# tphakala/go-audio-resampler

Hardware: AMD Instinct MI355X
Metric: Msamples/s resampled (float32, 44.1k→48k QualityHigh) + RMS error vs Go ref (higher is better)
Workload: dtype f32

## Files before the change

go-audio-resampler_amd/csrc/gar_hxs.hip:

```cpp
#include <hip/hip_runtime.h>

#include <algorithm>
#include <cstdio>
#include <cstdlib>
#include <utility>
#include <vector>

#include "gar_hxt.hpp"

namespace gar {

#define GAR_HXS_EXT(NS, V) extern template hipError_t hxsLaunch<NS, V>(const HxsArgs&, size_t, int64_t, hipStream_t);
GAR_HXS_FOR_ALL(GAR_HXS_EXT)
#undef GAR_HXS_EXT
#define GAR_HXT_EXT(NS, F, V, L) extern template hipError_t hxtLaunch<NS, F, V, L>(const HxsArgs&, size_t, int64_t, hipStream_t);
GAR_HXT_FOR_A(GAR_HXT_EXT)
GAR_HXT_FOR_B(GAR_HXT_EXT)
#undef GAR_HXT_EXT

namespace {
constexpr int kProfWords = 64 + 2 * 4096;
unsigned long long* profBuf() {
    static unsigned long long* p = nullptr;
    static bool init = false;
    if (!init) {
        init = true;
        if (std::getenv("GAR_HXS_PROF") && hipMalloc(&p, kProfWords * sizeof(unsigned long long)) == hipSuccess) {
            (void)hipMemset(p, 0, kProfWords * sizeof(unsigned long long));
            (void)hipMemset(p + 10, 0xff, sizeof(unsigned long long));
            (void)hipMemset(p + 13, 0xff, sizeof(unsigned long long));
            std::atexit([] {
                static unsigned long long h[kProfWords] = {};
                if (hipDeviceSynchronize() == hipSuccess && hipMemcpy(h, p, sizeof(h), hipMemcpyDeviceToHost) == hipSuccess) {
                    const double nl = h[3] ? static_cast<double>(h[3]) : 1, nc = h[6] ? static_cast<double>(h[6]) : 1;
                    fprintf(stderr, "hxs prof per wave (cycles): loaders convert %.0f issue+wait %.0f (issue %.0f) barrier %.0f (life %.1f us) | compute convert+mfma %.0f barrier %.0f\n",
                            h[0] / nl, h[1] / nl, h[7] / nl, h[2] / nl, h[9] / nl / 100.0, h[4] / nc, h[5] / nc);
                    fprintf(stderr, "hxs loader pre-loop %.2f us, post-loop %.2f us; compute convert %.0f\n", h[8] / nl / 100.0, h[12] / nl / 100.0, h[15] / nc);
                    if (h[23]) fprintf(stderr, "hxs wave-0 first block (cycles): entry->window %.0f, window->steps done %.0f, ->exit (stores drained) %.0f, n %llu\n",
                                       static_cast<double>(h[20]) / h[23], static_cast<double>(h[21]) / h[23], static_cast<double>(h[22]) / h[23], h[23]);
                    if (h[23]) fprintf(stderr, "hxs wave-0: entry->A landed %.0f, entry->barrier 1 %.0f; wave entry spread in a workgroup %.0f, wave 0 after first wave %.0f\n",
                                       static_cast<double>(h[24]) / h[23], static_cast<double>(h[25]) / h[23], static_cast<double>(h[26]) / h[23], static_cast<double>(h[27]) / h[23]);
                    if (h[34]) fprintf(stderr, "hxt roles per block (cycles): compute wave 0 %.0f (waiting %.0f), loader 0 %.0f (waiting %.0f), n %llu\n",
                                       static_cast<double>(h[30]) / h[34], static_cast<double>(h[32]) / h[34], static_cast<double>(h[31]) / h[34],
                                       static_cast<double>(h[33]) / h[34], h[34]);
                    if (h[34]) fprintf(stderr, "hxt compute wave 0: entry -> first group %.0f cycles, last group -> exit %.0f cycles, periods %.0f, arrivals %.0f\n",
                                       static_cast<double>(h[35]) / h[34], static_cast<double>(h[36]) / h[34],
                                       static_cast<double>(h[37]) / h[34], static_cast<double>(h[38]) / h[34]);
                    if (h[34] && h[57]) fprintf(stderr, "hxt fill (cycles): entry -> A issued %.0f, -> fill barrier %.0f, -> first group %.0f; in-kernel clock %.3f GHz\n",
                                       static_cast<double>(h[53]) / h[34], static_cast<double>(h[54]) / h[34], static_cast<double>(h[55]) / h[34],
                                       0.1 * static_cast<double>(h[56]) / static_cast<double>(h[57]));
                    if (h[34]) fprintf(stderr, "hxt loader 0 phases (cycles): load data wait %.0f, conversion %.0f, arrival %.0f\n",
                                       static_cast<double>(h[50]) / h[34], static_cast<double>(h[51]) / h[34], static_cast<double>(h[52]) / h[34]);
                    if (h[44]) fprintf(stderr, "hxq wave 0 (cycles): entry->barrier 1 %.0f, ->image %.0f, ->MFMA+stores issued %.0f, ->drained %.0f, n %llu\n",
                                       static_cast<double>(h[40]) / h[44], static_cast<double>(h[41]) / h[44], static_cast<double>(h[42]) / h[44],
                                       static_cast<double>(h[43]) / h[44], h[44]);
                    fprintf(stderr, "hxs span: first start -> last end %.1f us; loader wave life min %.1f max %.1f us\n",
                            (h[11] - h[10]) / 100.0, h[13] / 100.0, h[14] / 100.0);
                    std::vector<std::pair<double, int>> v;
                    unsigned long long t0 = ~0ull;
                    for (int b = 0; b < 4096; ++b)
                        if (h[65 + 2 * b]) { v.push_back({h[65 + 2 * b] / 100.0, b}); t0 = std::min(t0, h[64 + 2 * b]); }
                    if (!v.empty()) {
                        std::vector<std::pair<double, int>> sv = v;
                        std::sort(sv.begin(), sv.end());
                        auto pc = [&](double q) { return sv[std::min(sv.size() - 1, static_cast<size_t>(q * sv.size()))].first; };
                        fprintf(stderr, "hxs WG life us: n %zu min %.1f p10 %.1f p50 %.1f p90 %.1f max %.1f |", sv.size(), sv.front().first, pc(0.1), pc(0.5), pc(0.9), sv.back().first);
                        for (int m = 0; m < 8; ++m) {
                            double s = 0; int n = 0;
                            for (auto& e : v) if (e.second % 8 == m) { s += e.first; ++n; }
                            fprintf(stderr, " x%d %.1f", m, n ? s / n : 0.0);
                        }
                        fprintf(stderr, "\n  slowest:");
                        for (size_t k = sv.size(); k-- > 0 && k + 8 >= sv.size();)
                            fprintf(stderr, " b%d %.1fus@+%.1f", sv[k].second, sv[k].first, (h[64 + 2 * sv[k].second] - t0) / 100.0);
                        fprintf(stderr, "\n");
                    }
                }
            });
        }
    }
    return p;
}

int64_t fdiv(int64_t a, int64_t b) { return a >= 0 ? a / b : -((-a + b - 1) / b); }
int64_t cdiv(int64_t a, int64_t b) { return -fdiv(-a, b); }

template <int NS, int NL>
hipError_t hxtFmtL(const HxsArgs& x, size_t lds, int64_t blocks, hipStream_t st) {
    if (x.fmt == 1 && x.vst == 2) return hxtLaunch<NS, 1, 2, NL>(x, lds, blocks, st);
    if (x.fmt == 2 && x.vst == 0) return hxtLaunch<NS, 2, 0, NL>(x, lds, blocks, st);
    if (x.fmt == 2 && x.vst == 1) return hxtLaunch<NS, 2, 1, NL>(x, lds, blocks, st);
    if (x.fmt == 5 && x.vst == 0) return hxtLaunch<NS, 5, 0, NL>(x, lds, blocks, st);
    return hipErrorNotSupported;
}
template <int NS>
hipError_t hxtFmt(const HxsArgs& x, size_t lds, int64_t blocks, hipStream_t st) {
    return x.ncomp + 6 <= kHxtWaves ? hxtFmtL<NS, 6>(x, lds, blocks, st) : hxtFmtL<NS, 4>(x, lds, blocks, st);
}

static int hxtRoles(int nprog, int NS, int* role, int* maxStride) {
    static const int knobRoles = std::getenv("GAR_HXT_ROLES") ? std::atoi(std::getenv("GAR_HXT_ROLES")) : -1;
    const bool balanced = knobRoles >= 0 ? knobRoles != 0 : NS >= 10;
    int w = 0;
    *maxStride = 1;
    if (!balanced) {
        for (int i = 0; i < nprog; ++i) role[w++] = i | (1 << 16);
        return w;
    }
    const int q = nprog / 4 * 4, r = nprog - q;
    for (int i = 0; i < q; ++i) role[w++] = i | (1 << 16);
    if (r == 2 && q + 4 <= kHxtMaxComp) {
        for (int i = 0; i < 4; ++i) role[w++] = (q + (i & 1)) | ((i >> 1) << 8) | (2 << 16);
        *maxStride = 2;
    } else if (r == 1 && q + 4 <= kHxtMaxComp) {
        for (int i = 0; i < 4; ++i) role[w++] = q | (i << 8) | (4 << 16);
        *maxStride = 4;
    } else {
        for (int i = q; i < nprog; ++i) role[w++] = i | (1 << 16);
    }
    return w;
}

template <int NS>
hipError_t hxsVst(const HxsArgs& x, size_t lds, int64_t blocks, hipStream_t st) {
    switch (x.vst) {
        case 0: return hxsLaunch<NS, 0>(x, lds, blocks, st);
        case 1: return hxsLaunch<NS, 1>(x, lds, blocks, st);
        case 2: return hxsLaunch<NS, 2>(x, lds, blocks, st);
        case 4: return hxsLaunch<NS, 4>(x, lds, blocks, st);
        default: return hxsLaunch<NS, 3>(x, lds, blocks, st);
    }
}
}

static_assert(kHxtSyncOff + kHxtSyncBytes <= 320, "hxt progress counters past the reserved LDS");
static size_t hxsLds(int Rt) { return 4 * (16 * static_cast<size_t>(Rt) + 64) + 320; }
static_assert(288 + kHxtSyncBytes <= 448, "hxt FMT 5 progress counters past the reserved LDS");
static size_t hxtLdsWide(int Rt) { return 8 * (16 * static_cast<size_t>(Rt) + 64) + 448; }

static void hxsRingFor(const HxDev& p, int G, int& R, int& Rt, int& Wg) {
    const int GQ = G * p.Qc;
    Wg = (G - 1) * p.Qc + p.Kread;
    const int n = (Wg + GQ + GQ - 1) / GQ;
    R = n * GQ;
    Rt = (R + std::max(0, Wg - GQ) + 15) / 16 * 16;
}
constexpr size_t kHxsStaticLds = kHxsDev ? sizeof(unsigned long long) * kHxsWaves : 0;
static bool hxsRingFits(const HxDev& p, int G, int Rt) {
    return hxsLds(Rt) + kHxsStaticLds <= 160 * 1024 && (G * p.Qc + 63) / 64 <= kHxsNP;
}

static bool hxsNsBuilt(int ns) { return GAR_HXS_QUICK ? (ns == 9 || ns == 10) : (ns >= 1 && ns <= 10); }

bool hxsPlanFits(const HxDev& p) {
    if (!p.rb || p.nw > kHxRbMaxWaves || !hxsNsBuilt(p.NS)) return false;
// ... 31 lines not shown
        hxsRingFor(p, 2, r2, rt2, wg2);
        wide = ms == 1 && hxtLdsWide(rt2) <= 160 * 1024 && 2 * Qc <= hxtMaxRowsF(5, nc + 6 <= kHxtWaves ? 6 : 4) &&
               r2 / (2 * static_cast<int>(Qc)) + 3 <= kHxtSlots;
    }
    const int bw = wide ? 32 : 16;
    const int64_t targetBlocks = static_cast<int64_t>(ncu) * (knobWg > 0 ? knobWg : 1);
    const int64_t nchunkT = small ? nmac : std::max<int64_t>(1, (targetBlocks * bw + C - 1) / C);
    int64_t Np = std::max<int64_t>(1, cdiv(nmac, nchunkT));
    static const int knobNp = std::getenv("GAR_HXS_NP") ? std::atoi(std::getenv("GAR_HXS_NP")) : 0;
    if (knobNp > 0 && !small) Np = knobNp;
    const int inEsz = src.in_pcm ? pcmBytes(src.in_pcm) : (src.in_f64 ? 8 : 4);
    const int64_t rowBytes = std::max<int64_t>(4, src.in_fs * inEsz);
    const int64_t chunksPerRsrc = (C <= 16 && 16 % C == 0) ? 16 / C : 1;
    const int64_t npMax = ((int64_t(1) << 31) / rowBytes / chunksPerRsrc - (3 * Qc + p.Kread + 256)) / Qc;
    const bool rawSpan = npMax >= 1;
    if (rawSpan) Np = std::min(Np, npMax);
    int64_t nchunk = cdiv(nmac, Np);
    if (16 % C == 0 && !small) nchunk = cdiv(nchunk * C, 16) * 16 / C;
    const int64_t ncols = nchunk * C;
    if (ncols > (int64_t(1) << 30) || Np > (int64_t(1) << 24)) return hipErrorNotSupported;

    const uintptr_t inA = reinterpret_cast<uintptr_t>(src.in);
    int fmt = 0;
    const bool stereoIl = C == 2 && src.in_fs == 2 && src.in_cs == 1;
    if (!src.in) {
        const uintptr_t hA = reinterpret_cast<uintptr_t>(src.hist);
        if (C == 2 && src.hist_ld == 2 && (hA & 7) == 0) fmt = 1;
        else if (C % 16 == 0 && src.hist_ld % 4 == 0 && (hA & 15) == 0) fmt = 2;
    } else if (src.in_pcm == 16) {
        if ((inA & 3) == 0 && stereoIl) fmt = 3;
    } else if (src.in_pcm) {
        if ((inA & 7) == 0 && stereoIl) fmt = 4;
    } else if (src.in_f64) {
    } else if ((inA & 7) == 0 && stereoIl) {
        fmt = 1;
    } else if ((inA & 15) == 0 && C % 16 == 0 && src.in_cs == 1 && src.in_fs % 4 == 0) {
        fmt = 2;
    }
    const int esz = od.pcm ? pcmBytes(od.pcm) : (od.f64 ? 8 : 4);
    char* const outBase = reinterpret_cast<char*>(reinterpret_cast<uintptr_t>(od.out) - static_cast<uintptr_t>(od.o0 * od.fs * esz));
    const bool al = (reinterpret_cast<uintptr_t>(outBase) & 15) == 0;
    int vst;
    if (od.pcm == 16 && al && C == 2 && od.fs == 2 && od.cs == 1 && Pc % 4 == 0) vst = 4;
    else if (od.pcm) vst = 0;
    else if (od.f64) vst = 3;
    else if (al && C == 2 && od.fs == 2 && od.cs == 1 && Pc % 4 == 0) vst = 2;
    else if (al && od.fs == 1 && (od.cs * 4) % 16 == 0 && Pc % 4 == 0) vst = 1;
    else vst = 0;

    static const int knobHxt = std::getenv("GAR_HXT") ? std::atoi(std::getenv("GAR_HXT")) : -1;
    int role[kHxtMaxComp] = {}, maxStride = 1, ncomp = 0;
    bool hxt = knobHxt != 0 && !small && !od.pcm && !od.f64 && !src.in_pcm &&
               ((fmt == 1 && vst == 2) || (fmt == 2 && (vst == 0 || vst == 1)));
    if (hxt) ncomp = hxtRoles(p.nw, p.NS, role, &maxStride);
    wide = wide && hxt && fmt == 2 && vst == 0;
    if (wide) fmt = 5;

    int G = 0, R = 0, Rt = 0, Wg = 0;
    auto pickG = [&]() {
        for (int pass = hxt && maxStride > 1 ? 0 : 1; pass < 2 && G == 0; ++pass) {
            for (int cand = small ? 1 : kHxsMaxG; cand >= 1; --cand) {
                int r, rt, wg;
                hxsRingFor(p, cand, r, rt, wg);
                if (cand > 1 && cand > Np) continue;
                if (knobG > 0 && cand > knobG && cand > 1) continue;
                if (fmt == 5 ? hxtLdsWide(rt) > 160 * 1024 : !hxsRingFits(p, cand, rt)) continue;
                if (hxt && cand * Qc > hxtMaxRowsF(fmt, ncomp + 6 <= kHxtWaves ? 6 : 4)) continue;
                if (hxt && r / (cand * static_cast<int>(Qc)) + 3 > kHxtSlots) continue;
                if (pass == 0 && cand % maxStride != 0) continue;
                G = cand; R = r; Rt = rt; Wg = wg;
                break;
            }
        }
    };
    pickG();
    if (fmt == 5 && (G < 2 || maxStride > 1)) {
        fmt = 2;
        G = 0;
        pickG();
    }
    if (G == 0 && hxt) {
        hxt = false;
        ncomp = 0;
        maxStride = 1;
        for (int& r : role) r = 0;
        pickG();
    }
    if (G == 0) return hipErrorNotSupported;

    HxsArgs x{};
    x.A = static_cast<const h8v*>(p.A);
    x.progs = p.progs;
    x.ea = p.ea;
    x.Pc = p.Pc; x.Qc = p.Qc; x.Kc = p.Kc; x.Kread = p.Kread; x.G = G; x.C = C;
    x.nprog = p.nw;
    x.ncols = static_cast<int>(ncols);
    x.nblocks = static_cast<int>(fmt == 5 ? (ncols + 31) / 32 : (ncols + 15) / 16);
    x.Np = static_cast<int>(Np);
    x.ngroups = static_cast<int>(cdiv(Np, G));
    x.R = R; x.Rt = Rt; x.mirror = std::max(0, Wg - G * static_cast<int>(Qc)); x.Wg = Wg;
    x.a_lo = a_lo; x.a_hi = a_hi;
    x.dbg = knobDbg;
    x.prof = profBuf();
    x.o_lo = od.o_lo; x.o_hi = od.o_hi;
    const bool rawOk = src.in && fmt != 0 && src.in_len > 0 && src.in_fs > 0 && src.in_cs >= 0 && rawSpan;
    x.in_esz = inEsz;
    x.in_pcm = src.in_pcm;
    x.in = reinterpret_cast<const char*>(reinterpret_cast<uintptr_t>(src.in) -
                                         static_cast<uintptr_t>(src.in_base * src.in_fs * inEsz));
    x.in_fs = src.in_fs;
    x.in_cs = src.in_cs;
    x.fastLo = rawOk ? src.in_base : 0;
    x.fastHi = rawOk ? std::min(src.in_base + src.in_len, src.valid_end) : 0;
    x.fmt = fmt;
    x.small = small ? 1 : 0;
    static const int knobSmallK = std::getenv("GAR_HXS_SMALLK") ? std::atoi(std::getenv("GAR_HXS_SMALLK")) : 1;
    x.bigSmall = knobSmallK ? 0 : 1;
    static const int knobNt = std::getenv("GAR_HXS_NT") ? std::atoi(std::getenv("GAR_HXS_NT")) : 0;
    static const int knobPair = std::getenv("GAR_HXS_PAIR") ? std::atoi(std::getenv("GAR_HXS_PAIR")) : 1;
    x.nt = knobNt;
    x.xcdPair = knobPair && fmt == 2 && (C / 16) % 2 == 0 && x.nblocks % 16 == 0 ? 1 : 0;
    static const int knobChunkMajor = std::getenv("GAR_HXT_CHUNKMAJOR") ? std::atoi(std::getenv("GAR_HXT_CHUNKMAJOR")) : 1;
    if (knobChunkMajor && fmt == 5 && x.nblocks % 8 == 0) x.xcdPair = 2;
    x.out_pcm = od.pcm;
    x.out_f64 = od.f64;
    x.out = outBase;
    x.out_fs = od.fs * esz;
    x.out_cs = od.cs * esz;
    x.vst = vst;
    x.ncomp = ncomp;
    for (int w = 0; w < kHxtMaxComp; ++w) x.role[w] = role[w];
    x.err = od.err;
    x.pollMax = 1 << 24;
    x.faultNeed = 0;
    static const int knobCoop = std::getenv("GAR_HXT_COOP") ? std::atoi(std::getenv("GAR_HXT_COOP")) : 2;
    x.coop = std::max(0, std::min(2, knobCoop));
    if (hxt) {
        const char* f = std::getenv("GAR_HXT_FAULT");
        if (f && f[0] == '1') {
            x.pollMax = 1 << 12;
            x.faultNeed = 1 << 28;
        }
    }
    x.src = src;
    x.od = od;
    x.rows = p.rows;
    x.rowOff = p.rowOff;
    x.rowLen = p.rowLen;
    x.rowMax = p.rowMax;
    x.twoStage = p.twoStage;
    x.rowPh = p.rowPh;
    x.rowPar = p.rowPar;
    x.polyA = p.polyA;
    x.dftC = p.dftC;
    x.T1 = p.T1;
    x.T2 = p.T2;
    if (trace)
        fprintf(stderr, "%s: small=%d o[%lld,%lld) C=%d G=%d Np=%lld ngroups=%d nblocks=%d R=%d Rt=%d Wg=%d fmt=%d vst=%d fast[%lld,%lld)\n",
                hxt ? "hxt" : "hxs", x.small, (long long)od.o_lo, (long long)od.o_hi, C, G, (long long)Np, x.ngroups, x.nblocks, R, Rt, Wg, x.fmt, x.vst,
                (long long)x.fastLo, (long long)x.fastHi);
    if (hc && hc->n > 0 && hc->dst) {
        x.hdst = static_cast<float*>(hc->dst);
        x.ht0 = hc->t0;
        x.hn = hc->n;
        hc->done = true;
    }
    static const int knobHxq = std::getenv("GAR_HXQ") ? std::atoi(std::getenv("GAR_HXQ")) : 1;
    static const int knobHxqNr = std::getenv("GAR_HXQ_NR") ? std::atoi(std::getenv("GAR_HXQ_NR")) : 0;
    {
        const uintptr_t hA = reinterpret_cast<uintptr_t>(src.hist);
        const int hAl = fmt == 1 ? 8 : (fmt == 2 ? 16 : 4), hLd = fmt == 1 ? 2 : (fmt == 2 ? 4 : 1);
        const bool histOk = !src.hist || src.hist_len <= 0 ||
                            ((hA % hAl) == 0 && src.hist_ld % hLd == 0 && src.hist_len * src.hist_ld * 4 < (int64_t(1) << 31));
        const int64_t spanRows = (16 / C + 2) * Np * Qc + Wg;
        const bool gen = fmt == 0 && !src.in_pcm && src.in_fs >= 0 && src.in_cs >= 0 &&
                         (spanRows * src.in_fs + static_cast<int64_t>(C) * src.in_cs) * inEsz < (int64_t(1) << 31);
        const bool hkOk = !hc || hc->n <= 0 || (hc->n * src.in_fs + static_cast<int64_t>(C) * src.in_cs) * inEsz < (int64_t(1) << 31);
        if (small && knobHxq && ((fmt == 1 || fmt == 2) ? rawSpan : gen) && histOk && hkOk && p.nw <= 12 && x.Np == 1) {
            int nr = 1;
            for (int cand = p.nw; cand >= 1; --cand)
                if (x.nblocks * static_cast<int64_t>(cdiv(p.nw, cand)) >= static_cast<int64_t>(ncu)) { nr = cand; break; }
            if (knobHxqNr > 0) nr = std::min(knobHxqNr, p.nw);
            static const int knobOpt = std::getenv("GAR_HXQ_OPT") ? std::atoi(std::getenv("GAR_HXQ_OPT")) : 1;
            x.qOpt = knobOpt;
            x.qRbs = nr;
            x.qGroups = static_cast<int>(cdiv(p.nw, nr));
            for (int w = 0; w < p.nw; ++w) { x.qU0[w] = p.hU0[w]; x.qRbw[w] = p.hRbw[w]; }
            if (fmt == 0) {
                x.fastLo = src.in ? src.in_base : 0;
                x.fastHi = src.in ? std::min(src.in_base + src.in_len, src.valid_end) : 0;
            }
        }
    }
    if (small && !x.bigSmall) {
        Rt = R = (Wg + 15) / 16 * 16;
        x.R = R; x.Rt = Rt; x.mirror = 0;
    }
    if (trace && x.qGroups > 0) fprintf(stderr, "hxq: qRbs=%d qGroups=%d workgroups=%lld\n", x.qRbs, x.qGroups, (long long)x.nblocks * x.qGroups);
    const size_t lds = fmt == 5 ? hxtLdsWide(Rt) : hxsLds(Rt);
    const int64_t blocks = x.nblocks;
    if (hxt) {
        const int64_t hblocks = blocks;
        switch (p.NS) {
#define GAR_HXT_NS(n) case n: return hxtFmt<n>(x, lds, hblocks, stream);
#if !GAR_HXS_QUICK
            GAR_HXT_NS(1) GAR_HXT_NS(2) GAR_HXT_NS(3) GAR_HXT_NS(4) GAR_HXT_NS(5) GAR_HXT_NS(6) GAR_HXT_NS(7)
            GAR_HXT_NS(8)
#endif
            GAR_HXT_NS(9) GAR_HXT_NS(10)
#undef GAR_HXT_NS
            default: return hipErrorNotSupported;
        }
    }
    switch (p.NS) {
#define GAR_HXS_NS(n) case n: return hxsVst<n>(x, lds, blocks, stream);
#if !GAR_HXS_QUICK
        GAR_HXS_NS(1) GAR_HXS_NS(2) GAR_HXS_NS(3) GAR_HXS_NS(4) GAR_HXS_NS(5) GAR_HXS_NS(6) GAR_HXS_NS(7)
        GAR_HXS_NS(8)
#endif
        GAR_HXS_NS(9) GAR_HXS_NS(10)
#undef GAR_HXS_NS
        default: return hipErrorNotSupported;
    }
}

}
```

go-audio-resampler_amd/csrc/gar_hxt.hpp:

```cpp
#pragma once
#include "gar_hxs.hpp"

namespace gar {

constexpr int kHxtMaxComp = 12;
constexpr int kHxtWaves = 16;
constexpr int kHxtD = 2;
__host__ __device__ constexpr int hxtPieces(int NL) { return NL >= 6 ? 12 : 10; }
__host__ __device__ constexpr int hxtMaxRows(int NL) { return 64 * hxtPieces(NL); }
template <int NL>
constexpr int hxtItems() { return (4 * hxtPieces(NL) + NL - 1) / NL; }
__host__ __device__ constexpr int hxtQuads(int FMT) { return FMT == 5 ? 8 : 4; }
__host__ __device__ constexpr int hxtCols(int FMT) { return 4 * hxtQuads(FMT); }
__host__ __device__ constexpr int hxtMaxRowsF(int FMT, int NL) {
    return FMT == 5 ? 8 * NL * ((4 * hxtPieces(NL) + NL - 1) / NL) : 64 * hxtPieces(NL);
}
#ifndef GAR_HXT_CPRIO
#define GAR_HXT_CPRIO 0
#endif
#ifndef GAR_HXT_LPRIO
#define GAR_HXT_LPRIO 0
#endif
#ifndef GAR_HXT_CTDBG
#define GAR_HXT_CTDBG 0
// ... 284 lines not shown
    const int W = x.fmt == 5 ? 32 : 16;
    const bool blockLive = (x.fmt == 1 || x.fmt == 2 || x.fmt == 5) && b * W + W - 1 < x.ncols && x.fastHi > x.fastLo;
    const int64_t row0 = (x.a_lo + static_cast<int64_t>((b * W) / x.C) * x.Np) * x.Qc;
    return blockLive && row0 >= x.fastLo;
}

template <int FMT, int kCoopB, bool kOrdered>
__device__ __forceinline__ void hxtCoopStage0(const HxsArgs& x, const HxsShared& sh, int b, int w, int nw, int lane) {
    const HxsArgsP xp = hxsCold();
    const HxsRegSrc rs = hxsRegSrc<FMT>(xp, b, lane);
    HxsStage st;
    st.T0 = 0;
    st.nrow = x.Wg;
    st.fast = true;
    const int Wg = x.Wg;
    const int nit = FMT == 1 ? 4 * ((Wg + 63) >> 6) : FMT == 5 ? (Wg + 7) >> 3 : (Wg + 15) >> 4;
    bool met = !kOrdered;
    for (int it0 = w; it0 < nit; it0 += kCoopB * nw) {
        f32x4 e[kCoopB];
#pragma unroll
        for (int u = 0; u < kCoopB; ++u) {
            const int it = it0 + u * nw;
            const bool on = it < nit;
            if constexpr (FMT == 1) {
                const int q = it & 3, pc = it >> 2;
                const int o = on ? rs.lane0 + 64 * pc * rs.rowB + 2 * q * rs.chunkB : kHxqOob;
                const int o2 = on ? o + rs.chunkB : kHxqOob;
                const f2v a = __builtin_bit_cast(f2v, __builtin_amdgcn_raw_buffer_load_b64(rs.r, o, 0, 0));
                const f2v c = __builtin_bit_cast(f2v, __builtin_amdgcn_raw_buffer_load_b64(rs.r, o2, 0, 0));
                e[u] = f32x4{a.x, a.y, c.x, c.y};
            } else {
                const int o = on ? rs.lane0 + (FMT == 5 ? 8 : 16) * it * rs.rowB : kHxqOob;
                e[u] = __builtin_bit_cast(f32x4, __builtin_amdgcn_raw_buffer_load_b128(rs.r, o, 0, 0));
            }
        }
        if (!met) {
            hxsBarrier();
            met = true;
        }
#pragma unroll
        for (int u = 0; u < kCoopB; ++u) {
            const int it = it0 + u * nw;
            if (it >= nit) continue;
            const int q = FMT == 1 ? (it & 3) : FMT == 5 ? (lane & 7) : (lane >> 4);
            const int row = FMT == 1 ? 64 * (it >> 2) + lane : FMT == 5 ? 8 * it + (lane >> 3) : 16 * it + (lane & 15);
            if (row < Wg) hxsPutItem(xp, st, 0, q, row, e[u], sh.ring, sh.QS, sh.loudLo, sh.loudHi, sh.flag);
        }
    }
    if (!met) hxsBarrier();
}

template <int FMT, int NL>
__device__ __forceinline__ void hxtLoaders(const HxsArgs& x, const HxsShared& sh, const HxtSync& sy, int b, int l,
                                           int lane, int coop, unsigned long long* waited) {
    if constexpr (GAR_HXT_LPRIO > 0) __builtin_amdgcn_s_setprio(GAR_HXT_LPRIO);
    const HxsArgsP xp = hxsCold();
    const int GQ = x.G * x.Qc, Wg = x.Wg, R = x.R;
    const int P = (Wg + GQ - 1) / GQ, nL = P + x.ngroups - 1;
    const int nstepsPad = hxsStepsPad(x);
    const int dbg = kHxsDev ? x.dbg : GAR_HXT_CTDBG;
    const int c1 = b * hxtCols(FMT) + hxtCols(FMT) - 1;
    const bool blockLive = x.fmt >= 1 && x.fmt <= 5 && c1 < x.ncols && x.fastHi > x.fastLo;
    const int64_t row0 = (x.a_lo + static_cast<int64_t>((b * hxtCols(FMT)) / x.C) * x.Np) * x.Qc;
    const int64_t fastLo = x.fastLo;
    auto stage = [&](int j) {
        HxsStage st;
        st.T0 = j < P ? j * GQ : Wg + (j - P) * GQ;
        st.nrow = j < P ? min(GQ, Wg - j * GQ) : GQ;
        st.fast = blockLive && row0 + st.T0 >= fastLo;
        return st;
    };
    HxtBuf<FMT, NL> buf[kHxtD];
    bool fastL[kHxtD];
    const HxsRegSrc rs = hxsRegSrc<FMT>(xp, b, lane);
    const int jStart = coop ? P : 0;
    if (coop == 2) {
        hxsBarrier();
        fastL[0] = hxtIssue<FMT, NL>(stage(jStart), jStart < nL, rs, l, buf[0]);
        hxsBarrier();
#pragma unroll
        for (int d = 1; d < kHxtD; ++d) fastL[d] = hxtIssue<FMT, NL>(stage(jStart + d), jStart + d < nL, rs, l, buf[d]);
    } else {
#pragma unroll
        for (int d = 0; d < kHxtD; ++d) fastL[d] = hxtIssue<FMT, NL>(stage(jStart + d), jStart + d < nL, rs, l, buf[d]);
        if (coop) hxsBarrier();
    }
    int p0 = coop ? Wg : 0, last = Wg + GQ - 1 - R, need = 0;
    for (int j0 = jStart; j0 < nstepsPad; j0 += kHxtD) {
#pragma unroll
        for (int d = 0; d < kHxtD; ++d) {
            const int j = j0 + d;
            if (j < nL) {
                if (j >= P) {
                    if (j == P) p0 = Wg;
                    need = last < 0 ? 0 : need + 1;
                    if (need > 0 && !(dbg & 64)) hxtWait(x, sy, sy.cpArr, need - 1, x.ncomp, kHxtErrSlotWait, lane, waited);
                    last += GQ;
                }
                const bool stp = kHxsDev && waited;
                unsigned long long t1 = stp ? __builtin_amdgcn_s_memtime() : 0;
                if (stp && fastL[d]) {
                    constexpr int kNewer = (FMT == 1 ? 2 : 1) * hxtItems<NL>() * (kHxtD - 1);
                    static_assert(kNewer < 64, "vmcnt field");
                    __builtin_amdgcn_s_waitcnt((kNewer & 15) | (7 << 4) | (15 << 8) | ((kNewer >> 4) << 14));
                    const unsigned long long t2 = __builtin_amdgcn_s_memtime();
                    waited[3] += t2 - t1;
                    t1 = t2;
                }
                if (!((dbg & 16) && j >= P)) {
                    const HxsStage st = stage(j);
                    if (fastL[d]) hxtConvert<FMT, NL>(x, st, uni(p0), buf[d], b, l, lane, sh);
                    else hxtGatherLoad<hxtQuads(FMT)>(xp, st, b, l, NL, lane, sh);
                }
                unsigned long long t3 = stp ? __builtin_amdgcn_s_memtime() : 0;
                if (stp) waited[4] += t3 - t1;
                hxtArrive(sy.ldArr, j, lane);
                if (stp) waited[5] += __builtin_amdgcn_s_memtime() - t3;
                p0 += GQ;
                if (p0 >= R) p0 -= R;
            }
            fastL[d] = hxtIssue<FMT, NL>(stage(j + kHxtD), j + kHxtD < nL && !((dbg & 1) && j >= P), rs, l, buf[d]);
        }
    }
}

__device__ __forceinline__ int hxtBlock(const HxsArgs& x, int i) {
    if (x.xcdPair == 2) return (i & 7) * (x.nblocks >> 3) + (i >> 3);
    return hxsBlock(x, i);
}

#ifndef GAR_HXT_NTST2
#define GAR_HXT_NTST2 1
#endif
__device__ __forceinline__ void hxtStoreStereoNt(char* p, const f32x4& y, int lane) {
    const bool even = (lane & 1) == 0;
    const float s0 = even ? y[2] : y[0], s1 = even ? y[3] : y[1];
    const float q0 = __int_as_float(__builtin_amdgcn_mov_dpp(__float_as_int(s0), 0xB1, 0xf, 0xf, false));
    const float q1 = __int_as_float(__builtin_amdgcn_mov_dpp(__float_as_int(s1), 0xB1, 0xf, 0xf, false));
    f32x4 w;
    if (even) { w[0] = y[0]; w[1] = q0; w[2] = y[1]; w[3] = q1; }
    else      { w[0] = q0; w[1] = y[2]; w[2] = q1; w[3] = y[3]; }
    __builtin_nontemporal_store(w, reinterpret_cast<f32x4*>(p));
}

template <int NS, int VST, bool FAST, int NT = 1>
__device__ __forceinline__ void hxtGroups(const HxsArgs& x, const HxsShared& sh_, const HxtSync& sy, int wt, int lane,
                                          const h8v (&Ah)[NS], const h8v (&Al)[NS], uint32_t laneOff, int u0, int P,
                                          int nslot, const HxtRole& ro, char* obase, int64_t pstride, int64_t aCol,
                                          int64_t oRow0, bool colOk, int ccol, bool fullRb, int nl, unsigned long long* st) {
    const int sh = -(x.ea + kHxXs);
    const int GQ = x.G * x.Qc;
    const uint32_t dL = 8u * static_cast<uint32_t>(x.Rt);
    const uint32_t pst = 8u * static_cast<uint32_t>(x.Qc) * static_cast<uint32_t>(ro.st);
    const int dbg = kHxsDev ? x.dbg : GAR_HXT_CTDBG;
    const uint32_t tileLds = 4u * sh_.QS;
    const int64_t tileOut = 16 * x.out_cs;
    auto epilogue = [&](const f32x4& oA, const f32x4& oL, int p, int h) {
        const f32x4 y = hxScale(oA, oL, sh);
        if (dbg & 2) return;
        if constexpr (FAST && VST == 2 && GAR_HXT_NTST2) {
            hxtStoreStereoNt(obase + static_cast<int64_t>(p) * pstride, y, lane);
        } else if constexpr (FAST) {
            hxsStoreFast<VST>(x, obase + static_cast<int64_t>(p) * pstride + h * tileOut, y, lane);
        } else {
            const int ccol_ = ccol + 16 * h;
            const int64_t a = aCol + p;
            const int64_t o0 = a * x.Pc + oRow0;
            const bool live = colOk && a < x.a_hi;
            if (fullRb && live && a * x.Pc >= x.o_lo && (a + 1) * x.Pc <= x.o_hi) {
                char* pp = x.out + (o0 + ((VST == 2 && (lane & 1)) ? 2 : 0)) * x.out_fs + (VST == 2 ? 0 : ccol_ * x.out_cs);
                hxsStoreFast<VST>(x, pp, y, lane);
            } else if (live) {
#pragma unroll
                for (int i = 0; i < 4; ++i) {
                    const int64_t o = o0 + i;
                    if (oRow0 + i < x.Pc && o >= x.o_lo && o < x.o_hi)
                        *reinterpret_cast<float*>(x.out + o * x.out_fs + ccol_ * x.out_cs) = y[i];
                }
            }
        }
    };
    int first = ro.ph;
    for (int g = 0; g < x.ngroups; ++g) {
        const int p0 = g * x.G;
        const int pend = min(p0 + x.G, x.Np);
        while (first < p0) first += ro.st;
        const int n = first >= pend ? 0 : (pend - first + ro.st - 1) / ro.st;
        if (n > 0) {
            if (!(dbg & 32)) hxtWait(x, sy, sy.ldArr, P + g - 1 + x.faultNeed, nl, kHxtErrLoadWait, lane, st);
            if (kHxsDev && st) {
                const unsigned long long tg = __builtin_amdgcn_s_memtime();
                if (st[1] == 0) st[1] = tg;
                st[5] = tg;
            }
            int ln = lane;
            asm volatile("" : "+v"(ln));
            const uint32_t lo = ((ln & 15) & 3) * sh_.QS + 8u * (4 * (ln >> 4) + ((ln & 15) >> 2));
            uint32_t aH = static_cast<uint32_t>(reinterpret_cast<uintptr_t>((lds_s4p)(sh_.ring))) + lo + 8u * static_cast<uint32_t>(u0) +
                          8u * static_cast<uint32_t>((g % nslot) * GQ) + 8u * static_cast<uint32_t>(x.Qc) * static_cast<uint32_t>(first - p0);
            h8v bh0 = (dbg & 8) ? h8v{} : bFragA(aH), bl0 = (dbg & 8) ? h8v{} : bFragA(aH + dL);
            for (int i = 0; i < n; ++i) {
#pragma unroll
              for (int h = 0; h < NT; ++h) {
                asm volatile("" : "+v"(aH));
                const bool last = i + 1 == n && h + 1 == NT;
                uint32_t aL = aH + dL;
#if GAR_HXT_LOBASE
                asm volatile("" : "+v"(aL));
#endif
                const uint32_t aN = h + 1 < NT ? aH + tileLds : aH - (NT - 1) * tileLds + pst, aNL = aN + dL;
                f32x4 nA = {0, 0, 0, 0}, nL = nA;
#pragma unroll
                for (int s = 0; s < NS; ++s) {
// ... 23 lines not shown
        if (kHxsDev && st && n > 0) st[3] += ta - st[5];
        hxtArrive(sy.cpArr, g, lane);
        if (kHxsDev && st) st[4] += __builtin_amdgcn_s_memtime() - ta;
    }
    if (kHxsDev && st) st[2] = __builtin_amdgcn_s_memtime();
}

template <int NS, int VST, int FMT>
__device__ __forceinline__ void hxtCompute(const HxsArgs& x, const HxsShared& sh_, const HxtSync& sy, int b, int wt,
                                           int lane, int nl, int coop, unsigned long long* st) {
    if constexpr (GAR_HXT_CPRIO > 0) __builtin_amdgcn_s_setprio(GAR_HXT_CPRIO);
    const HxtRole ro = hxtRole(x, wt);
    const int* pt = x.progs + kBgProgInts * ro.rb;
    const int u0 = uni(pt[4]), rbw = uni(pt[3]);
    h8v Ah[NS], Al[NS];
#pragma unroll
    for (int i = 0; i < NS; ++i) {
        Ah[i] = x.A[((static_cast<size_t>(ro.rb) * NS + i) * 2 + 0) * 64 + lane];
        Al[i] = x.A[((static_cast<size_t>(ro.rb) * NS + i) * 2 + 1) * 64 + lane];
    }
    if (kHxsDev && st) st[6] = __builtin_amdgcn_s_memtime();
    if (coop) {
        if (coop == 2) hxtCoopStage0<FMT, 4, true>(x, sh_, b, wt, x.ncomp, lane);
        else hxtCoopStage0<FMT, 4, false>(x, sh_, b, wt, x.ncomp, lane);
        hxsBarrier();
    }
    if (kHxsDev && st) st[7] = __builtin_amdgcn_s_memtime();
    const uint32_t QS = sh_.QS;
    const int GQ = x.G * x.Qc;
    const int grp = lane >> 4, l16 = lane & 15;
    const uint32_t laneOff = (l16 & 3) * QS + 8u * (4 * grp + (l16 >> 2));
    const bool fullRb = (rbw + 1) * 16 <= x.Pc;
    const int nslot = x.R / GQ;
    const int P = (x.Wg + GQ - 1) / GQ;
    const int64_t pstride = static_cast<int64_t>(x.Pc) * x.out_fs;
    const int col = b * hxtCols(FMT) + l16;
    const bool colOk = col < x.ncols;
    const int kcol = col / x.C, ccol = col - kcol * x.C;
    const int64_t aCol = x.a_lo + static_cast<int64_t>(kcol) * x.Np;
    const int64_t oRow0 = static_cast<int64_t>(rbw) * 16 + 4 * grp;
    const bool laneFast = fullRb && colOk && aCol + x.Np <= x.a_hi && aCol * x.Pc >= x.o_lo &&
                          (aCol + x.Np) * x.Pc <= x.o_hi;
    char* obase = x.out + (aCol * x.Pc + oRow0 + ((VST == 2 && (lane & 1)) ? 2 : 0)) * x.out_fs +
                  (VST == 2 ? 0 : ccol * x.out_cs);
    constexpr int NT = FMT == 5 ? 2 : 1;
    if (__builtin_amdgcn_ballot_w64(!laneFast) == 0)
        hxtGroups<NS, VST, true, NT>(x, sh_, sy, wt, lane, Ah, Al, laneOff, u0, P, nslot, ro, obase, pstride, aCol, oRow0,
                                     colOk, ccol, fullRb, nl, st);
    else
        hxtGroups<NS, VST, false, NT>(x, sh_, sy, wt, lane, Ah, Al, laneOff, u0, P, nslot, ro, obase, pstride, aCol, oRow0,
                                      colOk, ccol, fullRb, nl, st);
}

template <int NS, int FMT, int VST, int NL>
__global__ __launch_bounds__(64 * kHxtWaves) void hxt_kernel(HxsArgs x) {
    extern __shared__ __attribute__((aligned(16))) unsigned char smem[];
    HxsShared s;
    s.stamp = nullptr;
    s.QS = 16u * static_cast<uint32_t>(x.Rt) + 64u;
    s.ring = reinterpret_cast<char*>(smem);
    constexpr int NQ = hxtQuads(FMT), NC = hxtCols(FMT);
    s.loudLo = reinterpret_cast<int*>(smem + NQ * static_cast<size_t>(s.QS));
    s.loudHi = s.loudLo + NC;
    s.flag = s.loudHi + NC;
    HxtSync sy;
    sy.ldArr = (lds_i32*)(smem + NQ * static_cast<size_t>(s.QS) + hxtSyncOff(FMT));
    sy.cpArr = sy.ldArr + kHxtSlots;
    sy.abort = sy.cpArr + kHxtSlots;
    const int lane = threadIdx.x & 63;
    const int wt = uni(threadIdx.x >> 6);
    const bool comp = wt < x.ncomp;
    if (threadIdx.x == 0) *sy.abort = 0;
    const bool stampW = kHxsDev && x.prof && lane == 0 && (wt == 0 || wt == x.ncomp);
    const unsigned long long tEntry = stampW ? __builtin_amdgcn_s_memtime() : 0;
    const unsigned long long rEntry = stampW ? __builtin_amdgcn_s_memrealtime() : 0;
    unsigned long long st[8] = {0, 0, 0, 0, 0, 0, 0, 0};
    unsigned long long tBlockEnd = 0;
    for (int bi = blockIdx.x; bi < x.nblocks; bi += gridDim.x) {
        const int b = hxtBlock(x, bi);
        __syncthreads();
        if (threadIdx.x < NC) {
            s.loudLo[threadIdx.x] = INT_MAX;
            s.loudHi[threadIdx.x] = -1;
        }
        const int GQb = x.G * x.Qc, Pb = (x.Wg + GQb - 1) / GQb;
        const int coop = hxtStage0Fast(x, b) ? x.coop : 0;
        if (threadIdx.x < 2 * kHxtSlots) sy.ldArr[threadIdx.x] = (coop && static_cast<int>(threadIdx.x) < Pb) ? NL : 0;
        if (threadIdx.x == 64) *s.flag = 0;
        __syncthreads();
        const bool first = bi == static_cast<int>(blockIdx.x);
        unsigned long long* stp = (stampW && first) ? st : nullptr;
        if (comp) hxtCompute<NS, VST, FMT>(x, s, sy, b, wt, lane, NL, coop, stp);
        else hxtLoaders<FMT, NL>(x, s, sy, b, wt - x.ncomp, lane, coop, stp);
        if (stampW && first) tBlockEnd = __builtin_amdgcn_s_memtime();
        __syncthreads();
        if (*s.flag) {
            __builtin_amdgcn_s_waitcnt(0);
            __syncthreads();
            hxsFixup(hxsCold(), (NC / 16) * b, s.loudLo, s.loudHi);
            if constexpr (NC == 32) hxsFixup(hxsCold(), 2 * b + 1, s.loudLo + 16, s.loudHi + 16);
        }
    }
    if (x.hn > 0) hxsHistKeep(x, static_cast<int64_t>(blockIdx.x) * blockDim.x + threadIdx.x,
                              static_cast<int64_t>(gridDim.x) * blockDim.x);
    if (stampW) {
        __builtin_amdgcn_s_waitcnt(0);
        const unsigned long long tExit = __builtin_amdgcn_s_memtime(), rExit = __builtin_amdgcn_s_memrealtime();
        if (wt == 0) {
            atomicAdd(x.prof + 30, tBlockEnd - tEntry);
            atomicAdd(x.prof + 32, st[0]);
            atomicAdd(x.prof + 37, st[3]);
            atomicAdd(x.prof + 38, st[4]);
            atomicAdd(x.prof + 34, 1ull);
            atomicAdd(x.prof + 35, st[1] ? st[1] - tEntry : 0ull);
            atomicAdd(x.prof + 36, tExit - (st[2] ? st[2] : tExit));
            atomicAdd(x.prof + 53, st[6] - tEntry);
            atomicAdd(x.prof + 54, st[7] - st[6]);
            atomicAdd(x.prof + 55, st[1] ? st[1] - st[7] : 0ull);
            atomicAdd(x.prof + 56, tExit - tEntry);
            atomicAdd(x.prof + 57, rExit - rEntry);
            atomicMin(x.prof + 10, rEntry);
            atomicMax(x.prof + 11, rExit);
            if (blockIdx.x < 4096) { x.prof[64 + 2 * blockIdx.x] = rEntry; x.prof[65 + 2 * blockIdx.x] = rExit - rEntry; }
        } else {
            atomicAdd(x.prof + 31, tBlockEnd - tEntry);
            atomicAdd(x.prof + 33, st[0]);
            atomicAdd(x.prof + 50, st[3]);
            atomicAdd(x.prof + 51, st[4]);
            atomicAdd(x.prof + 52, st[5]);
        }
    }
}

template <int NS, int FMT, int VST, int NL>
hipError_t hxtLaunch(const HxsArgs& x, size_t lds, int64_t blocks, hipStream_t st) {
    if (x.ncomp + NL > kHxtWaves) return hipErrorInvalidConfiguration;
    if (const size_t lim_ = setMaxLdsOnce(reinterpret_cast<const void*>(&hxt_kernel<NS, FMT, VST, NL>)); lim_ < lds) return ldsTooBig("hxt_kernel", lds, lim_);
    hipLaunchKernelGGL((hxt_kernel<NS, FMT, VST, NL>), dim3(static_cast<unsigned>(blocks)), dim3(64 * (x.ncomp + NL)), lds,
                       st, x);
    return hipGetLastError();
}

#define GAR_HXT_FOR3(M, NS) M(NS, 1, 2, 4) M(NS, 2, 0, 4) M(NS, 2, 1, 4) M(NS, 1, 2, 6) M(NS, 2, 0, 6) M(NS, 2, 1, 6) \
    M(NS, 5, 0, 4) M(NS, 5, 0, 6)
#if GAR_HXS_QUICK
#define GAR_HXT_FOR_A(M) GAR_HXT_FOR3(M, 9)
#define GAR_HXT_FOR_B(M) GAR_HXT_FOR3(M, 10)
#else
#define GAR_HXT_FOR_A(M) GAR_HXT_FOR3(M, 1) GAR_HXT_FOR3(M, 2) GAR_HXT_FOR3(M, 3) GAR_HXT_FOR3(M, 4) GAR_HXT_FOR3(M, 5) \
    GAR_HXT_FOR3(M, 6) GAR_HXT_FOR3(M, 7)
#define GAR_HXT_FOR_B(M) GAR_HXT_FOR3(M, 8) GAR_HXT_FOR3(M, 9) GAR_HXT_FOR3(M, 10)
#endif
#define GAR_HXT_INST(NS, F, V, L) template hipError_t hxtLaunch<NS, F, V, L>(const HxsArgs&, size_t, int64_t, hipStream_t);

}
```

Measured before the change: 454,800.

## Add compile-time specialized lean loader path for stereo f32 QualityHigh geometry

```diff
diff --git a/go-audio-resampler_amd/csrc/gar_hxs.hip b/go-audio-resampler_amd/csrc/gar_hxs.hip
--- a/go-audio-resampler_amd/csrc/gar_hxs.hip
+++ b/go-audio-resampler_amd/csrc/gar_hxs.hip
@@ -17,6 +17,9 @@
 GAR_HXT_FOR_A(GAR_HXT_EXT)
 GAR_HXT_FOR_B(GAR_HXT_EXT)
 #undef GAR_HXT_EXT
+#define GAR_HXT_EXT_LEAN(NS, F, V, L, E) extern template hipError_t hxtLaunch<NS, F, V, L, E>(const HxsArgs&, size_t, int64_t, hipStream_t);
+GAR_HXT_FOR_LEAN(GAR_HXT_EXT_LEAN)
+#undef GAR_HXT_EXT_LEAN
 
 namespace {
 constexpr int kProfWords = 64 + 2 * 4096;
@@ -86,7 +89,9 @@
 int64_t cdiv(int64_t a, int64_t b) { return -fdiv(-a, b); }
 
 template <int NS, int NL>
-hipError_t hxtFmtL(const HxsArgs& x, size_t lds, int64_t blocks, hipStream_t st) {
+hipError_t hxtFmtL(const HxsArgs& x, size_t lds, int64_t blocks, hipStream_t st, bool lean) {
+    if constexpr (NS == kHxtLeanNS)
+        if (lean && x.fmt == 1 && x.vst == 2) return hxtLaunch<NS, 1, 2, NL, 1>(x, lds, blocks, st);
     if (x.fmt == 1 && x.vst == 2) return hxtLaunch<NS, 1, 2, NL>(x, lds, blocks, st);
     if (x.fmt == 2 && x.vst == 0) return hxtLaunch<NS, 2, 0, NL>(x, lds, blocks, st);
     if (x.fmt == 2 && x.vst == 1) return hxtLaunch<NS, 2, 1, NL>(x, lds, blocks, st);
@@ -94,13 +99,20 @@
     return hipErrorNotSupported;
 }
 template <int NS>
-hipError_t hxtFmt(const HxsArgs& x, size_t lds, int64_t blocks, hipStream_t st) {
-    return x.ncomp + 6 <= kHxtWaves ? hxtFmtL<NS, 6>(x, lds, blocks, st) : hxtFmtL<NS, 4>(x, lds, blocks, st);
-}
-
-static int hxtRoles(int nprog, int NS, int* role, int* maxStride) {
-    static const int knobRoles = std::getenv("GAR_HXT_ROLES") ? std::atoi(std::getenv("GAR_HXT_ROLES")) : -1;
-    const bool balanced = knobRoles >= 0 ? knobRoles != 0 : NS >= 10;
+hipError_t hxtFmt(const HxsArgs& x, size_t lds, int64_t blocks, hipStream_t st, bool lean) {
+    return x.ncomp + 6 <= kHxtWaves ? hxtFmtL<NS, 6>(x, lds, blocks, st, lean) : hxtFmtL<NS, 4>(x, lds, blocks, st, lean);
+}
+
+template <int NL>
+bool hxtLeanGeoIs(const HxsArgs& x) {
+    using Geo = HxtLeanGeo<NL>;
+    return x.Qc == Geo::Qc && x.G == Geo::G && x.R == Geo::R && x.Rt == Geo::Rt && x.Wg == Geo::Wg && x.mirror == Geo::mirror;
+}
+
+static int hxtRoles(int nprog, int NS, int* role, int* maxStride, bool leanPlan = false) {
+    const char* envRoles = std::getenv("GAR_HXT_ROLES");
+    const int knobRoles = envRoles ? std::atoi(envRoles) : -1;
+    const bool balanced = knobRoles >= 0 ? knobRoles != 0 : (NS >= 10 || leanPlan);
     int w = 0;
     *maxStride = 1;
     if (!balanced) {
@@ -238,7 +250,13 @@
     int role[kHxtMaxComp] = {}, maxStride = 1, ncomp = 0;
     bool hxt = knobHxt != 0 && !small && !od.pcm && !od.f64 && !src.in_pcm &&
                ((fmt == 1 && vst == 2) || (fmt == 2 && (vst == 0 || vst == 1)));
-    if (hxt) ncomp = hxtRoles(p.nw, p.NS, role, &maxStride);
+    bool leanPlan = hxt && !kHxsDev && p.NS == kHxtLeanNS && Pc == kHxtLeanPc && Qc == HxtLeanGeo<4>::Qc && p.Kread == 420 &&
+                    p.nw == 10 && fmt == 1 && vst == 2 && src.in_fs == 2 && inEsz == 4 && Np >= HxtLeanGeo<4>::G;
+    if (leanPlan) {
+        const char* e = std::getenv("GAR_HXT_LEAN");
+        leanPlan = !e || std::atoi(e) != 0;
+    }
+    if (hxt) ncomp = hxtRoles(p.nw, p.NS, role, &maxStride, leanPlan);
     wide = wide && hxt && fmt == 2 && vst == 0;
     if (wide) fmt = 5;
 
@@ -341,10 +359,11 @@
     x.dftC = p.dftC;
     x.T1 = p.T1;
     x.T2 = p.T2;
+    const bool lean = leanPlan && hxt && (ncomp + 6 <= kHxtWaves ? hxtLeanGeoIs<6>(x) : hxtLeanGeoIs<4>(x));
     if (trace)
-        fprintf(stderr, "%s: small=%d o[%lld,%lld) C=%d G=%d Np=%lld ngroups=%d nblocks=%d R=%d Rt=%d Wg=%d fmt=%d vst=%d fast[%lld,%lld)\n",
+        fprintf(stderr, "%s: small=%d o[%lld,%lld) C=%d G=%d Np=%lld ngroups=%d nblocks=%d R=%d Rt=%d Wg=%d fmt=%d vst=%d fast[%lld,%lld) ncomp=%d lean=%d\n",
                 hxt ? "hxt" : "hxs", x.small, (long long)od.o_lo, (long long)od.o_hi, C, G, (long long)Np, x.ngroups, x.nblocks, R, Rt, Wg, x.fmt, x.vst,
-                (long long)x.fastLo, (long long)x.fastHi);
+                (long long)x.fastLo, (long long)x.fastHi, ncomp, lean ? 1 : 0);
     if (hc && hc->n > 0 && hc->dst) {
         x.hdst = static_cast<float*>(hc->dst);
         x.ht0 = hc->t0;
@@ -388,7 +407,7 @@
     if (hxt) {
         const int64_t hblocks = blocks;
         switch (p.NS) {
-#define GAR_HXT_NS(n) case n: return hxtFmt<n>(x, lds, hblocks, stream);
+#define GAR_HXT_NS(n) case n: return hxtFmt<n>(x, lds, hblocks, stream, lean);
 #if !GAR_HXS_QUICK
             GAR_HXT_NS(1) GAR_HXT_NS(2) GAR_HXT_NS(3) GAR_HXT_NS(4) GAR_HXT_NS(5) GAR_HXT_NS(6) GAR_HXT_NS(7)
             GAR_HXT_NS(8)
diff --git a/go-audio-resampler_amd/csrc/gar_hxt.hpp b/go-audio-resampler_amd/csrc/gar_hxt.hpp
--- a/go-audio-resampler_amd/csrc/gar_hxt.hpp
+++ b/go-audio-resampler_amd/csrc/gar_hxt.hpp
@@ -360,12 +360,12 @@
 
 template <int FMT, int NL>
 __device__ __forceinline__ void hxtLoaders(const HxsArgs& x, const HxsShared& sh, const HxtSync& sy, int b, int l,
-                                           int lane, int coop, unsigned long long* waited) {
+                                           int lane, int coop, unsigned long long* waited, int jStop = INT_MAX) {
     if constexpr (GAR_HXT_LPRIO > 0) __builtin_amdgcn_s_setprio(GAR_HXT_LPRIO);
     const HxsArgsP xp = hxsCold();
     const int GQ = x.G * x.Qc, Wg = x.Wg, R = x.R;
-    const int P = (Wg + GQ - 1) / GQ, nL = P + x.ngroups - 1;
-    const int nstepsPad = hxsStepsPad(x);
+    const int P = (Wg + GQ - 1) / GQ, nL = min(P + x.ngroups - 1, jStop);
+    const int nstepsPad = min(hxsStepsPad(x), jStop);
     const int dbg = kHxsDev ? x.dbg : GAR_HXT_CTDBG;
     const int c1 = b * hxtCols(FMT) + hxtCols(FMT) - 1;
     const bool blockLive = x.fmt >= 1 && x.fmt <= 5 && c1 < x.ncols && x.fastHi > x.fastLo;
@@ -432,6 +432,181 @@
     }
 }
 
+template <int QC, int G_, int KREAD>
+struct HxtGeo {
+    static constexpr int Qc = QC, G = G_, GQ = G_ * QC, Wg = (G_ - 1) * QC + KREAD;
+    static constexpr int nslot = (Wg + GQ + GQ - 1) / GQ, R = nslot * GQ;
+    static constexpr int mirror = Wg > GQ ? Wg - GQ : 0;
+    static constexpr int Rt = (R + mirror + 15) / 16 * 16;
+    static constexpr int P = (Wg + GQ - 1) / GQ;
+    static constexpr uint32_t QS = 16u * Rt + 64u, dL = 8u * Rt;
+    static constexpr int i0 = (R + 1 - Wg + GQ - 1) / GQ - 1;
+    static_assert(Wg > GQ && mirror < GQ && P % kHxtD == 0 && i0 >= 0, "lean loaders: ring shape");
+};
+template <int NL>
+using HxtLeanGeo = HxtGeo<147, NL >= 6 ? 5 : 4, 420>;
+constexpr int kHxtLeanPc = 160, kHxtLeanNS = 9;
+
+template <int NL>
+struct HxtLeanMap;
+template <>
+struct HxtLeanMap<6> {
+    static constexpr int kItems = 8, kMaxPcL = 5;
+    __host__ __device__ static constexpr int q(int k) { return k & 3; }
+    __host__ __device__ static constexpr int pcS(int k) { return 6 * (k >> 2); }
+    __device__ static int qL(int) { return 0; }
+    __device__ static int pcL(int l) { return l; }
+};
+template <>
+struct HxtLeanMap<4> {
+    static constexpr int kItems = 10, kMaxPcL = 0;
+    __host__ __device__ static constexpr int q(int) { return 0; }
+    __host__ __device__ static constexpr int pcS(int k) { return k; }
+    __device__ static int qL(int l) { return l; }
+    __device__ static int pcL(int) { return 0; }
+};
+
+typedef uint32_t u32x2v __attribute__((ext_vector_type(2)));
+typedef __attribute__((address_space(3))) u32x2v lds_u2;
+__device__ __forceinline__ void hxtLdsPut(uint32_t a, uint2 v) { *reinterpret_cast<lds_u2*>(a) = u32x2v{v.x, v.y}; }
+
+template <int NL, class Geo>
+__device__ GAR_HXT_SLOW_ATTR void hxtLoudLoadLean(HxsArgsP xp, int T0, int b, int l, int lane, HxsShared sh) {
+    using M = HxtLeanMap<NL>;
+    const SrcDesc src = kload(&xp->src);
+    HxsStage st;
+    st.T0 = T0;
+    st.nrow = Geo::GQ;
+    st.fast = true;
+    const int p0 = uni(T0 % xp->R);
+    for (int k = 0; k < M::kItems; ++k) {
+        const int row = 64 * (M::pcL(l) + M::pcS(k)) + lane, q = M::qL(l) + M::q(k);
+        if (row >= Geo::GQ) continue;
+        f32x4 e;
+#pragma unroll
+        for (int n = 0; n < 4; ++n) {
+            const int col = b * 16 + 4 * q + n;
+            const int kk = col / xp->C, c = col - kk * xp->C;
+            e[n] = hxsGather(src, hxsChunkRow(xp, kk, T0 + row), c, xp->A);
+        }
+        hxsPutItem(xp, st, p0, q, row, e, sh.ring, sh.QS, sh.loudLo, sh.loudHi, sh.flag);
+    }
+}
+
+template <int NL>
+__device__ __forceinline__ void hxtIssueLean(const HxsRegSrc& rs, uint32_t v0, uint32_t chunkB, HxtBuf<1, NL>& r) {
+    using M = HxtLeanMap<NL>;
+#pragma unroll
+    for (int k = 0; k < M::kItems; ++k) {
+        const uint32_t o = v0 + 2u * M::q(k) * chunkB + 512u * M::pcS(k);
+        r.a[k] = __builtin_bit_cast(f2v, __builtin_amdgcn_raw_buffer_load_b64(rs.r, static_cast<int>(o), 0, 0));
+        r.b[k] = __builtin_bit_cast(f2v, __builtin_amdgcn_raw_buffer_load_b64(rs.r, static_cast<int>(o + chunkB), 0, 0));
+    }
+}
+
+template <int NL, class Geo>
+__device__ __forceinline__ uint32_t hxtConvertLean(const HxtBuf<1, NL>& r, int slot, uint32_t rb, int laneRow) {
+    using M = HxtLeanMap<NL>;
+    constexpr int K = M::kItems, GQ = Geo::GQ, R = Geo::R, kMaxLaneRow = 64 * M::kMaxPcL + 63, kSplitChunk = 4;
+    const int p0 = (Geo::mirror + (slot + 1) * GQ) % R;
+    uint32_t m = 0;
+#pragma unroll
+    for (int k0 = 0; k0 < K; k0 += kSplitChunk) {
+        uint2 hv[kSplitChunk], lv[kSplitChunk];
+#pragma unroll
+        for (int u = 0; u < kSplitChunk; ++u) {
+            if (k0 + u >= K) break;
+            const f32x4 e = hxtItem<1, NL>(r, k0 + u);
+            m = max(m, max(max(hxtMag(e[0]), hxtMag(e[1])), max(hxtMag(e[2]), hxtMag(e[3]))));
+            hxSplit2(e[0], e[1], hv[u].x, lv[u].x);
+            hxSplit2(e[2], e[3], hv[u].y, lv[u].y);
+        }
+#pragma unroll
+        for (int u = 0; u < kSplitChunk; ++u) {
+            if (k0 + u >= K) break;
+            const int rowS = 64 * M::pcS(k0 + u);
+            const int pu = p0 + rowS;
+            const int wrapAt = R - pu;
+            const uint32_t a = rb + static_cast<uint32_t>(M::q(k0 + u)) * Geo::QS + 8u * static_cast<uint32_t>(pu);
+            if (rowS + kMaxLaneRow < GQ || laneRow < GQ - rowS) {
+                hxtLdsPut(a, hv[u]);
+                hxtLdsPut(a + Geo::dL, lv[u]);
+                if (wrapAt <= kMaxLaneRow && laneRow >= wrapAt) {
+                    hxtLdsPut(a - 8u * R, hv[u]);
+                    hxtLdsPut(a - 8u * R + Geo::dL, lv[u]);
+                }
+            }
+        }
+    }
+    return m;
+}
+
+template <class Geo>
+__device__ __forceinline__ int hxtLeanFrom(const HxsArgs& x, int b, int kU) {
+    const bool blockLive = b * 16 + 15 < x.ncols && x.fastHi > x.fastLo;
+    if (!blockLive) return INT_MAX;
+    const int64_t row0 = (x.a_lo + static_cast<int64_t>((b * 16) / x.C) * x.Np) * Geo::Qc;
+    const int64_t lack = x.fastLo - (row0 + Geo::Wg);
+    const int64_t i = lack <= 0 ? 0 : (lack + Geo::GQ - 1) / Geo::GQ;
+    const int64_t iu = (i + kU - 1) / kU * kU;
+    return iu > (1 << 28) ? INT_MAX : Geo::P + static_cast<int>(iu);
+}
+
+template <int NL, class Geo>
+__device__ __forceinline__ void hxtLoadersLean(const HxsArgs& x, const HxsShared& sh, const HxtSync& sy, int b, int l,
+                                               int lane, int coop, int jBegin, unsigned long long* waited) {
+    using M = HxtLeanMap<NL>;
+    static_assert(M::kItems == hxtItems<NL>() && 64 * (M::kMaxPcL + 1 + M::pcS(M::kItems - 1)) >= Geo::GQ, "lean items cover a load");
+    static_assert(kHxtD == 2, "two register buffers");
+    constexpr int GQ = Geo::GQ, P = Geo::P, kU = (Geo::nslot % 2 ? 2 : 1) * Geo::nslot;
+    if constexpr (GAR_HXT_LPRIO > 0) __builtin_amdgcn_s_setprio(GAR_HXT_LPRIO);
+    const HxsArgsP xp = hxsCold();
+    const int nL = P + x.ngroups - 1;
+    const int dbg = kHxsDev ? x.dbg : GAR_HXT_CTDBG;
+    const HxsRegSrc rs = hxsRegSrc<1>(xp, b, lane);
+    const uint32_t chunkB = static_cast<uint32_t>(rs.chunkB);
+    const int laneRow = 64 * M::pcL(l) + lane;
+    const uint32_t rb = static_cast<uint32_t>(reinterpret_cast<uintptr_t>((lds_s4p)(sh.ring))) +
+                        static_cast<uint32_t>(M::qL(l)) * Geo::QS + 8u * static_cast<uint32_t>(laneRow);
+    uint32_t vo = 8u * static_cast<uint32_t>(laneRow) + 2u * static_cast<uint32_t>(M::qL(l)) * chunkB +
+                  8u * static_cast<uint32_t>(Geo::Wg + (jBegin - P) * GQ);
+    int jI = jBegin;
+    HxtBuf<1, NL> buf[kHxtD];
+    auto issue = [&](HxtBuf<1, NL>& r) {
+        const bool live = jI < nL && !(dbg & 1);
+        hxtIssueLean<NL>(rs, live ? vo : 0x80000000u, chunkB, r);
+        vo += 8u * GQ;
+        ++jI;
+    };
+    if (coop == 2) {
+        hxsBarrier();
+        issue(buf[0]);
+        hxsBarrier();
+        issue(buf[1]);
+    } else {
+        issue(buf[0]);
+        issue(buf[1]);
+        if (coop) hxsBarrier();
+    }
+    for (int j0 = jBegin; j0 < nL; j0 += kU) {
+#pragma unroll
+        for (int u = 0; u < kU; ++u) {
+            const int j = j0 + u;
+            if (j < nL) {
+                const int need = j - P - Geo::i0 + 1;
+                if (need > 0 && !(dbg & 64)) hxtWait(x, sy, sy.cpArr, need - 1, x.ncomp, kHxtErrSlotWait, lane, waited);
+                if (!(dbg & 16)) {
+                    const uint32_t m = hxtConvertLean<NL, Geo>(buf[u % kHxtD], u % Geo::nslot, rb, laneRow);
+                    if (__builtin_expect(__builtin_amdgcn_ballot_w64(m >= kHxtLoudBits) != 0, 0))
+                        hxtLoudLoadLean<NL, Geo>(xp, Geo::Wg + (j - P) * GQ, b, l, lane, sh);
+                }
+                hxtArrive(sy.ldArr, j, lane);
+            }
+            issue(buf[u % kHxtD]);
+        }
+    }
+}
+
 __device__ __forceinline__ int hxtBlock(const HxsArgs& x, int i) {
     if (x.xcdPair == 2) return (i & 7) * (x.nblocks >> 3) + (i >> 3);
     return hxsBlock(x, i);
@@ -467,6 +642,7 @@
         const f32x4 y = hxScale(oA, oL, sh);
         if (dbg & 2) return;
         if constexpr (FAST && VST == 2 && GAR_HXT_NTST2) {
+            static_assert(NT == 1, "stereo frame-pair stores: one tile per period");
             hxtStoreStereoNt(obase + static_cast<int64_t>(p) * pstride, y, lane);
         } else if constexpr (FAST) {
             hxsStoreFast<VST>(x, obase + static_cast<int64_t>(p) * pstride + h * tileOut, y, lane);
@@ -596,7 +772,7 @@
                                       colOk, ccol, fullRb, nl, st);
 }
 
-template <int NS, int FMT, int VST, int NL>
+template <int NS, int FMT, int VST, int NL, int LEAN = 0>
 __global__ __launch_bounds__(64 * kHxtWaves) void hxt_kernel(HxsArgs x) {
     extern __shared__ __attribute__((aligned(16))) unsigned char smem[];
     HxsShared s;
@@ -635,7 +811,14 @@
         const bool first = bi == static_cast<int>(blockIdx.x);
         unsigned long long* stp = (stampW && first) ? st : nullptr;
         if (comp) hxtCompute<NS, VST, FMT>(x, s, sy, b, wt, lane, NL, coop, stp);
-        else hxtLoaders<FMT, NL>(x, s, sy, b, wt - x.ncomp, lane, coop, stp);
+        else if constexpr (LEAN != 0) {
+            static_assert(FMT == 1, "lean loaders: stereo f32 frames");
+            using Geo = HxtLeanGeo<NL>;
+            constexpr int kU = (Geo::nslot % 2 ? 2 : 1) * Geo::nslot;
+            const int jLean = coop ? Geo::P : hxtLeanFrom<Geo>(x, b, kU);
+            if (!coop) hxtLoaders<FMT, NL>(x, s, sy, b, wt - x.ncomp, lane, 0, stp, jLean);
+            if (jLean != INT_MAX) hxtLoadersLean<NL, Geo>(x, s, sy, b, wt - x.ncomp, lane, coop, jLean, stp);
+        } else hxtLoaders<FMT, NL>(x, s, sy, b, wt - x.ncomp, lane, coop, stp);
         if (stampW && first) tBlockEnd = __builtin_amdgcn_s_memtime();
         __syncthreads();
         if (*s.flag) {
@@ -676,11 +859,11 @@
     }
 }
 
-template <int NS, int FMT, int VST, int NL>
+template <int NS, int FMT, int VST, int NL, int LEAN = 0>
 hipError_t hxtLaunch(const HxsArgs& x, size_t lds, int64_t blocks, hipStream_t st) {
     if (x.ncomp + NL > kHxtWaves) return hipErrorInvalidConfiguration;
-    if (const size_t lim_ = setMaxLdsOnce(reinterpret_cast<const void*>(&hxt_kernel<NS, FMT, VST, NL>)); lim_ < lds) return ldsTooBig("hxt_kernel", lds, lim_);
-    hipLaunchKernelGGL((hxt_kernel<NS, FMT, VST, NL>), dim3(static_cast<unsigned>(blocks)), dim3(64 * (x.ncomp + NL)), lds,
+    if (const size_t lim_ = setMaxLdsOnce(reinterpret_cast<const void*>(&hxt_kernel<NS, FMT, VST, NL, LEAN>)); lim_ < lds) return ldsTooBig("hxt_kernel", lds, lim_);
+    hipLaunchKernelGGL((hxt_kernel<NS, FMT, VST, NL, LEAN>), dim3(static_cast<unsigned>(blocks)), dim3(64 * (x.ncomp + NL)), lds,
                        st, x);
     return hipGetLastError();
 }
@@ -696,5 +879,7 @@
 #define GAR_HXT_FOR_B(M) GAR_HXT_FOR3(M, 8) GAR_HXT_FOR3(M, 9) GAR_HXT_FOR3(M, 10)
 #endif
 #define GAR_HXT_INST(NS, F, V, L) template hipError_t hxtLaunch<NS, F, V, L>(const HxsArgs&, size_t, int64_t, hipStream_t);
-
-}
+#define GAR_HXT_FOR_LEAN(M) M(kHxtLeanNS, 1, 2, 6, 1) M(kHxtLeanNS, 1, 2, 4, 1)
+#define GAR_HXT_INST_LEAN(NS, F, V, L, E) template hipError_t hxtLaunch<NS, F, V, L, E>(const HxsArgs&, size_t, int64_t, hipStream_t);
+
+}
diff --git a/go-audio-resampler_amd/csrc/gar_hxt_i3.hip b/go-audio-resampler_amd/csrc/gar_hxt_i3.hip
--- /dev/null
+++ b/go-audio-resampler_amd/csrc/gar_hxt_i3.hip
@@ -0,0 +1,5 @@
+#include "gar_hxt.hpp"
+
+namespace gar {
+GAR_HXT_FOR_LEAN(GAR_HXT_INST_LEAN)
+}
```

Result: faster. 462,200, median of 6 (+1.6%).
